# SensorsINI/v2e

Hardware: AMD Instinct MI355X
Metric: Mevents/s (EventEmulator.generate_events, 346x260, 10x slowdown) (higher is better)
Workload: dtype f64

## Files before the change

v2e_amd/csrc/emu.hip:

```cpp
#include "common.h"
#include "../../include/v2e_detmath.h"

#include <cstdarg>
#include <cstdlib>
#include <chrono>
#include <vector>

namespace {

constexpr int BLOCK = 256;
constexpr int WAVE = 64;
constexpr int RING = 64;
constexpr int SCAN_BLOCKS = 64;
constexpr int STAMP_LAUNCHES = 128;

constexpr uint32_t CNT_MASK = 0x00FFFFFFu;
constexpr uint32_t CNT_NEG = 1u << 24;
constexpr uint32_t CNT_SHOT_ON = 1u << 25;
constexpr uint32_t CNT_SHOT_OFF = 1u << 26;

struct FrameCtl {
    double t_prev, t_frame;
    double dt_over_tau;
    double shot_base;
// ... 1801 lines not shown
    const RunScratch &r = h->cur();
    const size_t esz = dtype == V2E_DT_U8 ? 1 : (dtype == V2E_DT_F32 ? 4 : 8);
    const bool has_refr = p->refractory_period_s > 0;
    const int K = h->ch_K, E = h->ch_E, m = E / K, D = h->ch_D, NC = h->n_clips, nD = h->ch_nD;
    const bool fused_rec = h->ch_fused != 0;
    const std::vector<ChainLaunch> plan = chain_plan(n_frames, K, E, nD, has_refr, fused_rec);
    const int nL = (int)plan.size();
    const int nB = (n_frames + K - 1) / K;
    const int nEB = (n_frames + E - 1) / E;
    KArgs a = a_in;
    Sched sc;
    sc.h = h; sc.st[ST_MAIN] = s; sc.st[ST_AHEAD] = h->ahead; sc.st[ST_SIDE] = h->side; sc.st[ST_TAB] = h->tabs; sc.st[ST_SIDE2] = h->side2;
    if (mode == ChainMode::profiled)
        for (int q = 0; q < ST_COUNT; ++q) sc.st[q] = s;
    auto mark = [&](bool rows, hipStream_t stq) -> int {
        if (mode != ChainMode::profiled) return 0;
        hipEvent_t e;
        V2E_HIP(hipEventCreate(&e));
        (rows ? marks->rows : marks->chain).push_back(e);
        V2E_HIP(hipEventRecord(e, stq));
        return 0;
    };
    int gy = NC;
    if (has_refr && K > 1) gy = std::max(1, std::min(NC, h->ch_max_blocks / std::max(h->ngroups, 1)));
    dim3 grid(h->ngroups, gy);
    const int tab_stream = captured || pipelined ? ST_SIDE : ST_TAB;
    constexpr int NSET = 3;
    auto launch_emission = [&](int b, int ef0, int enE) -> int {
        CEmitArgs ea;
        memset(&ea, 0, sizeof(ea));
        ea.ctl = r.run_ctl; ea.recs = recs; ea.fidx_base = r.run_fidx;
        ea.f0 = ef0; ea.nE = enE; ea.D = D; ea.n_clips = NC; ea.slot0 = ef0 % D;
        ea.nwp = h->ch_nwp; ea.nwaves = chain_egroups(h); ea.E = E;
        ea.cnt = r.ch_cnt; ea.tsold = has_refr ? r.ch_tsold : nullptr; ea.ruleM = has_refr ? r.ch_ruleM : nullptr;
        const size_t set = (size_t)(b % NSET) * E * NC;
        ea.wmax = r.ch_wmax + set * h->ch_nwp; ea.wtot = r.ch_wtot + set * h->nkeys_cap * h->ch_nwp;
        ea.cf = r.ch_cf + set; ea.cT = r.ch_cT + set * h->nkeys_cap; ea.ckbase = r.ch_ckbase + set * h->nkeys_cap;
        ea.cperm = r.ch_cperm + set * h->max_iters * 8; ea.cpre = r.ch_cpre + set * h->nkeys_cap * h->ch_nwp;
        ea.cdone = r.ch_cdone + set;
        const bool pull = r.ch_cmask != nullptr;
        ea.cmask = pull ? r.ch_cmask + set * h->ch_nwp * h->nkeys_cap * 2 * GPX : nullptr;
        bool two = h->ch_nwp > 1024;
        if (const char *ev = getenv("V2E_AMD_PULL_TWO_LEVEL")) two = atoi(ev) != 0;
        ea.cpre16 = pull && two ? r.ch_cpre16 + set * h->nkeys_cap * (h->ch_nwp / 16) : nullptr;
        ea.wpf = std::max(4, std::min(two ? 128 : 64, h->npx / (two ? 2048 : V2E_PULL_PX_PER_WG)));
        ea.p2 = two ? 16 : 64;
        while (ea.p2 < (two ? h->ch_nwp / 16 : ea.nwaves)) ea.p2 *= 2;
        ea.events = (float4 *)events; ea.cap = cap;
        ea.off_in = r.run_off + (size_t)b * NC;
        ea.off_out = r.run_off + (size_t)(b + 1) * NC;
        ea.ich = 4;
        ea.capw = GROUP_PX * ea.ich;
        ea.coff_in_cemit = captured || pipelined ? 1 : 0;
        ea.zpw_tot = CTOT_ZF;
        ea.zpw_emit = 1;
        const int REC_LDS = (ea.capw + WAVE) * 4 * (BLOCK / WAVE);
        const int egx = (chain_egroups(h) + BLOCK / WAVE - 1) / (BLOCK / WAVE);
        void *args[] = {(void *)&a, (void *)&ea};
        if (sc.wait(tab_stream, EV_FORK, b)) return V2E_EHIP;
        if (b >= NSET && !captured && sc.wait(tab_stream, EV_JOIN, b - NSET)) return V2E_EHIP;
        if (sc.kernel(tab_stream, (const void *)k_ctot, dim3(egx, NC, (ea.nE + CTOT_ZF - 1) / CTOT_ZF), dim3(BLOCK), 0, args)) return V2E_EHIP;
        if (h->ch_nwp <= 4096) {
            if (sc.kernel(tab_stream, (const void *)k_cframe1, dim3(1, NC, ea.nE), dim3(CFRAME_THREADS), 0, args)) return V2E_EHIP;
        } else if (sc.kernel(tab_stream, (const void *)k_cframe, dim3(std::min(h->nkeys_cap, CFRAME_ROWS), NC, ea.nE), dim3(CFRAME_THREADS), 0, args)) {
            return V2E_EHIP;
        }
        const int row_stream = pipelined ? ST_SIDE2 : captured ? ST_SIDE : ((b & 1) ? ST_SIDE2 : ST_SIDE);
        if (!ea.coff_in_cemit) {
            void *oargs[] = {(void *)&ea};
            if (sc.kernel(tab_stream, (const void *)k_coff, dim3(NC), dim3(WAVE), 0, oargs)) return V2E_EHIP;
        }
        if (sc.record(EV_TAB, b, tab_stream)) return V2E_EHIP;
        if (!captured && sc.wait(row_stream, EV_TAB, b)) return V2E_EHIP;
        if (mark(true, sc.st[row_stream])) return V2E_EHIP;
        if (pull) {
            if (sc.kernel(row_stream, ea.cpre16 ? (const void *)k_cpull<true> : (const void *)k_cpull<false>, dim3(8 * ea.wpf * ((ea.nE + 7) / 8), NC), dim3(BLOCK), (size_t)(2 * ea.p2 * (ea.cpre16 ? 4 : 6)), args)) return V2E_EHIP;
        } else if (sc.kernel(row_stream, (const void *)k_cemit, dim3(egx, NC, ea.nE), dim3(BLOCK), (size_t)REC_LDS, args)) return V2E_EHIP;
        if (mark(true, sc.st[row_stream])) return V2E_EHIP;
        return sc.record(EV_JOIN, b, row_stream);
    };
    const bool split0 = m > 1 && n_frames > K && !pipelined;
    const bool ahead_whole = pipelined && !fused_rec && n_frames <= D;
    auto launch_ahead = [&](int b) -> int {
        if (!ahead_whole && b >= nD && sc.wait(ST_AHEAD, EV_CHAIN, (b - nD + 1) * m)) return V2E_EHIP;
        const int b0 = ahead_whole ? 0 : b * E, b1 = ahead_whole ? n_frames : std::min((b + 1) * E, n_frames);
        const int cut = (b == 0 && split0) ? std::min(K, b1) : b1;
        for (int part = 0; part < 2; ++part) {
            const int f0 = part == 0 ? b0 : cut, f1 = part == 0 ? cut : b1;
            if (f1 <= f0) continue;
            AheadArgs aa;
            memset(&aa, 0, sizeof(aa));
            aa.frames_pp = r.run_frames; aa.frame_stride = (unsigned long long)NC * h->npx * esz;
            aa.ctl = r.run_ctl; aa.fidx_base = r.run_fidx;
            aa.f0 = f0; aa.nf = f1 - f0; aa.D = D; aa.n_clips = NC; aa.slot0 = f0 % D;
            aa.rec = r.ch_rec;
            {
                const int pairs = aa.nf / 2 + 1;
                const long long wg_xy = (long long)h->ngroups * NC;
                int zb = (int)std::min<long long>(pairs, std::max<long long>((4ll * h->n_cu + wg_xy - 1) / wg_xy, (pairs + 15) / 16));
                aa.ppt = (pairs + zb - 1) / zb;
            }
            void *args[] = {(void *)&a, (void *)&aa};
            if (sc.kernel(ST_AHEAD, (const void *)k_ahead<uint8_t>, dim3(h->ngroups, NC, (aa.nf / 2 + 1 + aa.ppt - 1) / aa.ppt), dim3(BLOCK), 0, args)) return V2E_EHIP;
            if (sc.record(EV_AHEAD, part == 0 ? b : nL, ST_AHEAD)) return V2E_EHIP;
        }
        return 0;
    };
    void *xb[2] = {h->base, has_refr ? h->ch_base2 : h->base}, *xl[2] = {h->lp, has_refr ? h->ch_lp2 : h->lp};
    float *xt[2] = {h->ts_mem, has_refr ? h->ch_ts2 : h->ts_mem};
    {
        void *const zp[4] = {recs, r.run_off, has_refr ? (void *)r.ch_gM : nullptr, has_refr ? (void *)r.ch_bar : nullptr};
        const size_t zb[4] = {sizeof(v2e_frame_rec) * (size_t)n_frames * NC, sizeof(unsigned long long) * NC,
                              sizeof(uint32_t) * (size_t)nL * (K + 1) * NC * K, sizeof(unsigned) * (size_t)nL * 2 * K * NC};
        if (sc.zero4(pipelined ? ST_AHEAD : ST_MAIN, zp, zb)) return V2E_EHIP;
    }
    if (!pipelined) {
        if (sc.record(EV_FORK, nL, ST_MAIN)) return V2E_EHIP;
        if (!captured && sc.wait(ST_SIDE, EV_FORK, nL)) return V2E_EHIP;
        if (!fused_rec && sc.wait(ST_AHEAD, EV_FORK, nL)) return V2E_EHIP;
// ... 570 lines not shown
```

v2e_amd/csrc/emu_chain.h:

```cpp
#pragma once
#include <type_traits>
#include "pull_index.h"

#ifndef V2E_CHAIN_LOCKSTEP
#define V2E_CHAIN_LOCKSTEP 0
#endif
#ifndef V2E_CHAIN_STAMPS
#define V2E_CHAIN_STAMPS 0
#endif

constexpr int CHAIN_K_MAX = 64;
constexpr int CFRAME_THREADS = 1024;
constexpr int CHAIN_SUB = 8;
constexpr int CHAIN_MAX_ITERS = 1024;

template <typename R> __device__ __forceinline__ R floor_div_pos(R a, R b)
{
    if (!(b > (R)0) || !(a >= (R)0)) return div_floor<R>(a, b);
    if (a < b) return (R)0;
    R q = floor(a / b);
    R r = fma(-q, b, a);
    if (r < (R)0) q -= (R)1;
    else if (r >= b) q += (R)1;
    return q;
}

__device__ __forceinline__ bool clip_barrier(unsigned *ctr, unsigned target, bool light = false)
{
    __shared__ int s_ok;
    asm volatile("s_waitcnt vmcnt(0)" ::: "memory");
    __syncthreads();
    if (threadIdx.x == 0) {
        if (!light) {
            __builtin_amdgcn_fence(__ATOMIC_RELEASE, "agent");
            asm volatile("s_waitcnt vmcnt(0)" ::: "memory");
        }
        __hip_atomic_fetch_add(ctr, 1u, __ATOMIC_RELAXED, __HIP_MEMORY_SCOPE_AGENT);
        unsigned spins = 0;
        int ok = 1;
        while (__hip_atomic_load(ctr, __ATOMIC_RELAXED, __HIP_MEMORY_SCOPE_AGENT) < target) {
            if (light) __builtin_amdgcn_s_sleep(1); else __builtin_amdgcn_s_sleep(4);
            if (++spins > 2000000u) { ok = 0; break; }
        }
        if (!light) __builtin_amdgcn_fence(__ATOMIC_ACQUIRE, "agent");
        s_ok = ok;
    }
    __syncthreads();
    return s_ok != 0;
}

struct FrameTab {
    float start, step, end;
    uint32_t refr_mask;
    __device__ __forceinline__ FrameTab(const FrameCtl *c, int lane)
        : start(c->ts_start[lane & 31]), step(c->ts_stepf[lane & 31]), end(c->ts_end), refr_mask(c->refr_mask) {}
// ... 616 lines not shown
                if (lane >= c0 && lane < fn) WT_STORE(&ca.ruleM[(size_t)sl * ca.n_clips + clip], rule_v);
            }
            if (own) break;
            if (valid) {
                ((R *)ca.base_fix)[sp] = b;
                if (lp_state) ((R *)ca.lp_fix)[sp] = lp;
                ca.ts_fix[sp] = tsm;
            }
            if (last_exact >= ca.pnf - 1) continue;
            __builtin_amdgcn_s_setprio(0);
            const bool ok = clip_barrier(ca.bar_prev + (size_t)bar_idx * ca.n_clips + clip, (unsigned)ca.ngroups, ca.bar_light != 0);
            ++bar_idx;
            if (ca.prio) __builtin_amdgcn_s_setprio(3);
            if (!ok && tid == 0) atomicOr(&ca.recs[(size_t)ca.pf0 * ca.n_clips + clip].flags, V2E_FLAG_SYNC_TIMEOUT);
        }
        if (valid && (ca.nf > 0 || ca.store_out || redone)) {
            ((R *)ca.base_out)[sp] = b;
            if (ca.nf > 0 || lp_state) ((R *)ca.lp_out)[sp] = lp;
            if (a.has_refr) ca.ts_out[sp] = tsm;
        }
        V2E_STAMP_C(15);
    }
    if (stamp && tid == 0) atomicMax(stamp + 2 * ca.lidx + 1, wall_clock64());
}

struct CFrame {
    int M;
    uint32_t n_events, n_signal, discarded;
};

struct CEmitArgs {
    const FrameCtl *ctl;
    v2e_frame_rec *recs;
    const uint32_t *fidx_base;
    int f0, nE, D, n_clips, nwp, nwaves, E;
    int slot0;
    const uint32_t *cnt;
    const uint32_t *ruleM;
    uint16_t *wmax;
    uint16_t *wtot;
    const float *tsold;
    CFrame *cf;
    uint32_t *cT;
    uint32_t *ckbase;
    uint32_t *cperm;
    uint32_t *cpre;
    float4 *events;
    unsigned long long cap;
    const unsigned long long *off_in;
    unsigned long long *off_out;
    unsigned *cdone;
    int capw, ich;
    int zpw_tot, zpw_emit;
    int coff_in_cemit;
    uint32_t *cmask;
    int wpf, p2;
    uint32_t *cpre16;
};

#ifndef V2E_GPX
#define V2E_GPX 4
#endif
constexpr int GPX = V2E_GPX;
constexpr int GROUP_PX = GPX * WAVE;
constexpr int GROUP_SRC_BITS = GPX <= 4 ? 8 : (GPX <= 8 ? 9 : 10);

constexpr int CTOT_ZF = 2;

__global__ __launch_bounds__(BLOCK) void k_ctot(KArgs a, CEmitArgs ea)
{
    const int tid = threadIdx.x, lane = tid & (WAVE - 1), wave = tid / WAVE;
    const int clip = blockIdx.y;
    const int grp = blockIdx.x * (BLOCK / WAVE) + wave;
    if (grp >= ea.nwaves) return;
    const int p0 = grp * GROUP_PX + lane;
    const int zb = (int)blockIdx.z * CTOT_ZF;
    uint32_t cwq[CTOT_ZF][GPX], rMq[CTOT_ZF];
    int slotq[CTOT_ZF];
    {
        int sl = ea.slot0 + zb;
        if (sl >= ea.D) sl -= ea.D;
#pragma unroll
        for (int q = 0; q < CTOT_ZF; ++q) {
            slotq[q] = sl;
            rMq[q] = 0u;
#pragma unroll
            for (int j = 0; j < GPX; ++j) {
                cwq[q][j] = 0u;
                if (zb + q < ea.nE && p0 + j * WAVE < a.npx) cwq[q][j] = ea.cnt[((size_t)sl * ea.n_clips + clip) * a.npx_pad + p0 + j * WAVE];
            }
            if (zb + q < ea.nE && ea.ruleM) rMq[q] = ea.ruleM[(size_t)sl * ea.n_clips + clip];
            if (++sl == ea.D) sl = 0;
        }
    }
#pragma unroll
    for (int q = 0; q < CTOT_ZF; ++q) {
        const int z = zb + q;
        if (z >= ea.nE) break;
        const size_t zc = (size_t)z * ea.n_clips + clip;
        const uint32_t rM = (uint32_t)__builtin_amdgcn_readfirstlane((int)rMq[q]);
        int magv[GPX];
        bool neg[GPX];
        unsigned long long negb[GPX];
        int mmax = 0;
        uint32_t son = 0, soff = 0;
        unsigned long long sob[GPX], sfb[GPX];
#pragma unroll
        for (int j = 0; j < GPX; ++j) {
            const uint32_t cw = cwq[q][j];
            magv[j] = (int)(cw & CNT_MASK);
            neg[j] = (cw & CNT_NEG) != 0;
            negb[j] = __ballot(neg[j]);
            mmax = max(mmax, magv[j]);
            sob[j] = __ballot((cw & CNT_SHOT_ON) != 0);
            sfb[j] = __ballot((cw & CNT_SHOT_OFF) != 0);
            son += (uint32_t)__popcll(sob[j]);
            soff += (uint32_t)__popcll(sfb[j]);
        }
        const int wm = wave_max_i32(mmax);
        if (lane == 0) ea.wmax[zc * ea.nwp + grp] = (uint16_t)min(wm, 65535);
        uint16_t *trow = ea.wtot + (zc * a.nkeys_cap) * ea.nwp + grp;
        uint32_t *mrow = ea.cmask ? ea.cmask + ((zc * a.nkeys_cap + (lane >= 2 * GPX ? 1 : 0)) * ea.nwp + grp) * (2 * GPX) + (lane & (2 * GPX - 1)) : nullptr;
        auto put_masks = [&](const int key_on, const unsigned long long (&on_m)[GPX], const unsigned long long (&off_m)[GPX]) __attribute__((always_inline)) {
            uint32_t mw = 0u;
#pragma unroll
            for (int j = 0; j < GPX; ++j) {
                asm("v_writelane_b32 %0, %1, %2" : "+v"(mw) : "s"((uint32_t)on_m[j]), "n"(2 * j));
                asm("v_writelane_b32 %0, %1, %2" : "+v"(mw) : "s"((uint32_t)(on_m[j] >> 32)), "n"(2 * j + 1));
                asm("v_writelane_b32 %0, %1, %2" : "+v"(mw) : "s"((uint32_t)off_m[j]), "n"(2 * GPX + 2 * j));
                asm("v_writelane_b32 %0, %1, %2" : "+v"(mw) : "s"((uint32_t)(off_m[j] >> 32)), "n"(2 * GPX + 2 * j + 1));
            }
            if (lane < 4 * GPX) mrow[(size_t)key_on * ea.nwp * (2 * GPX)] = mw;
        };
        static_assert(4 * GPX == 16, "k_ctot: the mask words of an iteration are one 16-lane DPP row");
        uint32_t pmask = 0u;
        if (mrow) {
#pragma unroll
            for (int j = 0; j < GPX; ++j) {
                asm("v_writelane_b32 %0, %1, %2" : "+v"(pmask) : "s"((uint32_t)negb[j]), "n"(2 * j));
                asm("v_writelane_b32 %0, %1, %2" : "+v"(pmask) : "s"((uint32_t)(negb[j] >> 32)), "n"(2 * j + 1));
                asm("v_writelane_b32 %0, %1, %2" : "+v"(pmask) : "s"((uint32_t)negb[j]), "n"(2 * GPX + 2 * j));
                asm("v_writelane_b32 %0, %1, %2" : "+v"(pmask) : "s"((uint32_t)(negb[j] >> 32)), "n"(2 * GPX + 2 * j + 1));
            }
            pmask = lane < 2 * GPX ? ~pmask : (lane < 4 * GPX ? pmask : 0u);
        }
        const int wmc = min(wm, a.max_iters);
        const int nkw = 2 + 2 * wmc;
        bool ruled = false;
        TsGen tg(0.f, 0.f, 0.f, 1);
        float tsm[GPX];
#pragma unroll
        for (int j = 0; j < GPX; ++j) tsm[j] = 0.f;
        if (rM != 0u) {
            const FrameCtl *c = ea.ctl + (size_t)(ea.f0 + z) * ea.n_clips + clip;
            const FrameTab ftb(c, lane);
            tg = frame_tsgen(a, c, ftb, (int)rM, ruled);
            if (ea.tsold) {
#pragma unroll
                for (int j = 0; j < GPX; ++j)
                    if (p0 + j * WAVE < a.npx) tsm[j] = ea.tsold[((size_t)slotq[q] * ea.n_clips + clip) * a.npx_pad + p0 + j * WAVE];
            }
        }
        for (int kb = 0; kb < nkw; kb += WAVE) {
            uint32_t mine = 0;
            const int i_lo = kb == 0 ? 0 : (kb - 2) / 2;
            const int i_hi = min((kb + WAVE - 2) / 2, wmc);
            uint32_t *mrow_i = mrow ? mrow + (size_t)(2 + 2 * i_lo) * ea.nwp * (2 * GPX) : nullptr;
            for (int i = i_lo; i < i_hi; ++i) {
                unsigned long long cb[GPX];
                if (!ruled) {
#pragma unroll
                    for (int j = 0; j < GPX; ++j) cb[j] = __ballot(magv[j] > i);
                } else {
#pragma unroll
                    for (int j = 0; j < GPX; ++j) {
                        bool pass = magv[j] > i;
                        if (pass) {
                            const float t = tg(i);
                            const float pt = 1.0f * t - tsm[j];
                            pass = pt > a.refr_f;
                            if (pass) tsm[j] = t;
                        }
                        cb[j] = __ballot(pass);
                    }
                }
                uint32_t on, off;
                if (mrow) {
                    uint32_t mw = 0u;
#pragma unroll
                    for (int j = 0; j < GPX; ++j) {
                        asm("v_writelane_b32 %0, %1, %2" : "+v"(mw) : "s"((uint32_t)cb[j]), "n"(2 * j));
                        asm("v_writelane_b32 %0, %1, %2" : "+v"(mw) : "s"((uint32_t)(cb[j] >> 32)), "n"(2 * j + 1));
                    }
                    mw = (uint32_t)__builtin_amdgcn_update_dpp((int)mw, (int)mw, 0x118, 0xf, 0xc, false) & pmask;
                    if (lane < 4 * GPX) *mrow_i = mw;
                    mrow_i += (size_t)2 * ea.nwp * (2 * GPX);
                    int c = __popc(mw);
                    c += V2E_DPP(c, 0x111);
                    c += V2E_DPP(c, 0x112);
                    c += V2E_DPP(c, 0x114);
                    on = (uint32_t)__builtin_amdgcn_readlane(c, 2 * GPX - 1);
                    off = (uint32_t)__builtin_amdgcn_readlane(c, 4 * GPX - 1);
                } else {
                    on = 0u;
                    off = 0u;
#pragma unroll
                    for (int j = 0; j < GPX; ++j) {
                        on += (uint32_t)__popcll(cb[j] & ~negb[j]);
                        off += (uint32_t)__popcll(cb[j] & negb[j]);
                    }
                }
                const int kl = 2 + 2 * i - kb;
                if (lane == kl) mine = on;
                if (lane == kl + 1) mine = off;
            }
            if (kb == 0) {
                if (lane == 0) mine = son;
                if (lane == 1) mine = soff;
                if (mrow && (son | soff) != 0u) put_masks(0, sob, sfb);
            }
            if (kb + lane < nkw) trow[(size_t)(kb + lane) * ea.nwp] = (uint16_t)mine;
        }
    }
}

__device__ __forceinline__ void key_row16(const uint16_t *__restrict__ row_at, const uint16_t *__restrict__ wm_at, uint32_t k, uint32_t v[16])
{
    const uint4 t0 = *(const uint4 *)row_at, t1 = *(const uint4 *)(row_at + 8);
    const uint4 m0 = *(const uint4 *)wm_at, m1 = *(const uint4 *)(wm_at + 8);
    const uint32_t tw[8] = {t0.x, t0.y, t0.z, t0.w, t1.x, t1.y, t1.z, t1.w};
    const uint32_t mw[8] = {m0.x, m0.y, m0.z, m0.w, m1.x, m1.y, m1.z, m1.w};
#pragma unroll
    for (int j = 0; j < 16; ++j) {
        const uint32_t wmj = (mw[j >> 1] >> (16 * (j & 1))) & 0xFFFFu;
        v[j] = k < 2u + 2u * wmj ? ((tw[j >> 1] >> (16 * (j & 1))) & 0xFFFFu) : 0u;
    }
}

__global__ __launch_bounds__(CFRAME_THREADS) void k_cframe1(KArgs a, CEmitArgs ea)
{
    __shared__ int s_red[CFRAME_THREADS / WAVE];
    __shared__ uint32_t s_T[2 * CHAIN_MAX_ITERS + 2];
    constexpr int NW = CFRAME_THREADS / WAVE;
    const int tid = threadIdx.x, lane = tid & (WAVE - 1), wave = tid / WAVE;
    const int clip = blockIdx.y, z = blockIdx.z, fe = ea.f0 + z;
    const uint16_t *wm = ea.wmax + ((size_t)z * ea.n_clips + clip) * ea.nwp;
    int m = 0;
    for (int k = tid; k < ea.nwaves; k += CFRAME_THREADS) m = max(m, (int)wm[k]);
    m = wave_max_i32(m);
    if (lane == 0) s_red[wave] = m;
    __syncthreads();
    int M = 0;
#pragma unroll
    for (int q = 0; q < NW; ++q) M = max(M, s_red[q]);
    M = __builtin_amdgcn_readfirstlane(M);
    CFrame *cf = ea.cf + (size_t)z * ea.n_clips + clip;
    v2e_frame_rec *rec = ea.recs + (size_t)fe * ea.n_clips + clip;
    if (M > a.max_iters) {
        if (tid == 0) {
            cf->M = M; cf->n_events = 0u; cf->n_signal = 0u; cf->discarded = 1u;
            rec->max_events = M;
            atomicOr(&rec->flags, V2E_FLAG_ITERS_CLAMPED);
        }
        return;
    }
    const int nk = 2 + 2 * M;
    const uint16_t *tot = ea.wtot + ((size_t)z * ea.n_clips + clip) * a.nkeys_cap * ea.nwp;
    uint32_t *pre = ea.cpre + ((size_t)z * ea.n_clips + clip) * a.nkeys_cap * ea.nwp;
    for (int k = wave; k < nk; k += NW) {
        uint32_t carry = 0;
        for (int w0 = 0; w0 < ea.nwp; w0 += 16 * WAVE) {
            const int wi = w0 + lane * 16;
            uint32_t v[16];
#pragma unroll
            for (int j = 0; j < 16; ++j) v[j] = 0u;
            if (wi < ea.nwp) {
                key_row16(tot + (size_t)k * ea.nwp + wi, wm + wi, (uint32_t)k, v);
            }
            uint32_t lane_tot = 0;
#pragma unroll
            for (int j = 0; j < 16; ++j) lane_tot += v[j];
            uint32_t run = carry + wave_excl_scan_u32(lane_tot, lane);
            carry += wave_sum_u32(lane_tot);
            if (wi < ea.nwp) {
                uint32_t o[16];
#pragma unroll
                for (int j = 0; j < 16; ++j) { o[j] = run; run += v[j]; }
                uint4 *dst = (uint4 *)(pre + (size_t)k * ea.nwp + wi);
                if (ea.cpre16) ea.cpre16[(((size_t)z * ea.n_clips + clip) * a.nkeys_cap + k) * (ea.nwp / 16) + wi / 16] = o[0];
                dst[0] = make_uint4(o[0], o[1], o[2], o[3]);
                dst[1] = make_uint4(o[4], o[5], o[6], o[7]);
                dst[2] = make_uint4(o[8], o[9], o[10], o[11]);
                dst[3] = make_uint4(o[12], o[13], o[14], o[15]);
            }
        }
        if (lane == 0) s_T[k] = carry;
    }
    __syncthreads();
    if (wave != 0) return;
    uint32_t *cT = ea.cT + ((size_t)z * ea.n_clips + clip) * a.nkeys_cap;
    uint32_t *ckb = ea.ckbase + ((size_t)z * ea.n_clips + clip) * a.nkeys_cap;
    uint32_t carry = 0, sum_on = 0, sum_off = 0;
    for (int kb = 0; kb < nk; kb += WAVE) {
        const int key = kb + lane;
        const uint32_t T_k = key < nk ? s_T[key] : 0u;
        const uint32_t sig = key >= 2 ? T_k : 0u;
        const uint32_t kbase = carry + wave_excl_scan_u32(sig, lane);
        if (key < a.nkeys_cap) { cT[key] = T_k; ckb[key] = kbase; }
        sum_on += wave_sum_u32((lane & 1) ? 0u : sig);
        sum_off += wave_sum_u32((lane & 1) ? sig : 0u);
        carry += wave_sum_u32(sig);
    }
    const uint32_t n_signal = carry;
    uint32_t *perm = ea.cperm + ((size_t)z * ea.n_clips + clip) * a.max_iters * 8;
    if (a.shuffle && a.rng_mode == V2E_RNG_PHILOX) {
        const uint32_t fbase = ea.fidx_base ? *ea.fidx_base : 0u;
        for (int i = lane; i < M; i += WAVE) {
            uint32_t pk[4], sh, aa, amask;
            const uint32_t n_i = s_T[2 + 2 * i] + s_T[3 + 2 * i];
            v2e_perm_shape(n_i, &sh, &aa, &amask);
            v2e_perm_keys(a.seed, (uint32_t)clip, fbase + (uint32_t)fe, (uint32_t)i, pk);
            uint4 *pp = (uint4 *)(perm + (size_t)i * 8);
            pp[0] = make_uint4(pk[0], pk[1], pk[2], pk[3]);
            pp[1] = make_uint4(sh, aa, amask, n_i);
        }
    }
    if (lane == 0) {
        const uint32_t son = a.do_shot ? s_T[0] : 0u, soff = a.do_shot ? s_T[1] : 0u;
        cf->M = M; cf->n_signal = n_signal; cf->n_events = n_signal + son + soff; cf->discarded = 0u;
        rec->max_events = M;
        rec->n_signal = n_signal;
        rec->n_events = n_signal + son + soff;
        rec->n_on = sum_on + son;
        rec->n_off = sum_off + soff;
    }
}

constexpr int CFRAME_ROWS = 24;

__global__ __launch_bounds__(CFRAME_THREADS) void k_cframe(KArgs a, CEmitArgs ea)
{
    constexpr int NW = CFRAME_THREADS / WAVE;
    __shared__ int s_red[NW];
    __shared__ uint32_t s_seg[NW];
    __shared__ uint32_t s_T[2 * CHAIN_MAX_ITERS + 2];
    __shared__ int s_last;
    const int tid = threadIdx.x, lane = tid & (WAVE - 1), wave = tid / WAVE;
    const int r0 = blockIdx.x, clip = blockIdx.y, z = blockIdx.z, fe = ea.f0 + z;
    const size_t zc = (size_t)z * ea.n_clips + clip;
    const uint16_t *wm = ea.wmax + ((size_t)z * ea.n_clips + clip) * ea.nwp;
    int m = 0;
    for (int k = tid; k < ea.nwaves; k += CFRAME_THREADS) m = max(m, (int)wm[k]);
    m = wave_max_i32(m);
    if (lane == 0) s_red[wave] = m;
    __syncthreads();
    int M = 0;
#pragma unroll
    for (int q = 0; q < NW; ++q) M = max(M, s_red[q]);
    M = __builtin_amdgcn_readfirstlane(M);
    CFrame *cf = ea.cf + zc;
    v2e_frame_rec *rec = ea.recs + (size_t)fe * ea.n_clips + clip;
    const bool discard = M > a.max_iters;
    const int nk = discard ? 0 : 2 + 2 * M;
    const uint16_t *tot = ea.wtot + ((size_t)z * ea.n_clips + clip) * a.nkeys_cap * ea.nwp;
    uint32_t *pre = ea.cpre + zc * a.nkeys_cap * ea.nwp;
    uint32_t *cT = ea.cT + zc * a.nkeys_cap;
    const int seg = ((ea.nwp + NW - 1) / NW + 15) / 16 * 16;
    for (int k = r0; k < nk; k += (r0 == (int)gridDim.x - 1 ? 1 : nk)) {
        const int lo = wave * seg, hi = min(lo + seg, ea.nwp);
        uint32_t wsum = 0;
        for (int w0 = lo; w0 < hi; w0 += 16 * WAVE) {
            const int wi = w0 + lane * 16;
            uint32_t lane_tot = 0;
            if (wi < hi) {
                uint32_t v[16];
                key_row16(tot + (size_t)k * ea.nwp + wi, wm + wi, (uint32_t)k, v);
#pragma unroll
                for (int j = 0; j < 16; ++j) lane_tot += v[j];
            }
            wsum += wave_sum_u32(lane_tot);
        }
        __syncthreads();
        if (lane == 0) s_seg[wave] = wsum;
        __syncthreads();
        uint32_t carry = 0, total = 0;
#pragma unroll
        for (int q = 0; q < NW; ++q) {
// ... 475 lines not shown
```

Baseline: 20120.

## Fuse per-frame table build into k_ctot via last-arrival counter and adaptive z-chunking

```diff
diff --git a/v2e_amd/csrc/ctot_walk.h b/v2e_amd/csrc/ctot_walk.h
--- /dev/null
+++ b/v2e_amd/csrc/ctot_walk.h
@@ -0,0 +1,23 @@
+#pragma once
+
+#if defined(__HIPCC__)
+#define V2E_CW_HD __host__ __device__ __forceinline__
+#else
+#define V2E_CW_HD static inline
+#endif
+
+#define CTOT_WG_GROUPS 4
+
+V2E_CW_HD int ctot_arrivals(int nwaves) { return (nwaves + CTOT_WG_GROUPS - 1) / CTOT_WG_GROUPS; }
+V2E_CW_HD int ctot_chunks(int nE, int zf) { return (nE + zf - 1) / zf; }
+V2E_CW_HD int ctot_chunk_frames(int nE, int zf, int c) { return nE - c * zf < zf ? nE - c * zf : zf; }
+V2E_CW_HD int ctot_slot(int slot0, int z, int D) { return slot0 + z >= D ? slot0 + z - D : slot0 + z; }
+V2E_CW_HD int ctot_next_slot(int sl, int D) { return sl + 1 == D ? 0 : sl + 1; }
+
+#define CTOT_ZF_MAX 16
+V2E_CW_HD int ctot_plan_zf(long long wgs_xy, int nE, int n_cu)
+{
+    int zf = CTOT_ZF_MAX;
+    while (zf > 1 && wgs_xy * ctot_chunks(nE, zf) < (long long)n_cu) zf /= 2;
+    return zf;
+}
diff --git a/v2e_amd/csrc/emu.hip b/v2e_amd/csrc/emu.hip
--- a/v2e_amd/csrc/emu.hip
+++ b/v2e_amd/csrc/emu.hip
@@ -1877,19 +1877,17 @@
         ea.ich = 4;
         ea.capw = GROUP_PX * ea.ich;
         ea.coff_in_cemit = captured || pipelined ? 1 : 0;
-        ea.zpw_tot = CTOT_ZF;
+        const int egx = ctot_arrivals(chain_egroups(h));
+        ea.zpw_tot = ctot_plan_zf((long long)egx * NC, ea.nE, h->n_cu);
+        if (const char *ev = getenv("V2E_AMD_CTOT_ZF")) { const int v = atoi(ev); if (v >= 1 && v <= 64) ea.zpw_tot = v; }
+        ea.fuse_frame = h->ch_nwp <= 4096 ? 1 : 0;
         ea.zpw_emit = 1;
         const int REC_LDS = (ea.capw + WAVE) * 4 * (BLOCK / WAVE);
-        const int egx = (chain_egroups(h) + BLOCK / WAVE - 1) / (BLOCK / WAVE);
         void *args[] = {(void *)&a, (void *)&ea};
         if (sc.wait(tab_stream, EV_FORK, b)) return V2E_EHIP;
         if (b >= NSET && !captured && sc.wait(tab_stream, EV_JOIN, b - NSET)) return V2E_EHIP;
-        if (sc.kernel(tab_stream, (const void *)k_ctot, dim3(egx, NC, (ea.nE + CTOT_ZF - 1) / CTOT_ZF), dim3(BLOCK), 0, args)) return V2E_EHIP;
-        if (h->ch_nwp <= 4096) {
-            if (sc.kernel(tab_stream, (const void *)k_cframe1, dim3(1, NC, ea.nE), dim3(CFRAME_THREADS), 0, args)) return V2E_EHIP;
-        } else if (sc.kernel(tab_stream, (const void *)k_cframe, dim3(std::min(h->nkeys_cap, CFRAME_ROWS), NC, ea.nE), dim3(CFRAME_THREADS), 0, args)) {
-            return V2E_EHIP;
-        }
+        if (sc.kernel(tab_stream, (const void *)k_ctot, dim3(egx, NC, ctot_chunks(ea.nE, ea.zpw_tot)), dim3(BLOCK), 0, args)) return V2E_EHIP;
+        if (!ea.fuse_frame && sc.kernel(tab_stream, (const void *)k_cframe, dim3(std::min(h->nkeys_cap, CFRAME_ROWS), NC, ea.nE), dim3(CFRAME_THREADS), 0, args)) return V2E_EHIP;
         const int row_stream = pipelined ? ST_SIDE2 : captured ? ST_SIDE : ((b & 1) ? ST_SIDE2 : ST_SIDE);
         if (!ea.coff_in_cemit) {
             void *oargs[] = {(void *)&ea};
diff --git a/v2e_amd/csrc/emu_chain.h b/v2e_amd/csrc/emu_chain.h
--- a/v2e_amd/csrc/emu_chain.h
+++ b/v2e_amd/csrc/emu_chain.h
@@ -1,6 +1,7 @@
 #pragma once
 #include <type_traits>
 #include "pull_index.h"
+#include "ctot_walk.h"
 
 #ifndef V2E_CHAIN_LOCKSTEP
 #define V2E_CHAIN_LOCKSTEP 0
@@ -723,6 +724,7 @@
     unsigned *cdone;
     int capw, ich;
     int zpw_tot, zpw_emit;
+    int fuse_frame;
     int coff_in_cemit;
     uint32_t *cmask;
     int wpf, p2;
@@ -736,165 +738,6 @@
 constexpr int GROUP_PX = GPX * WAVE;
 constexpr int GROUP_SRC_BITS = GPX <= 4 ? 8 : (GPX <= 8 ? 9 : 10);
 
-constexpr int CTOT_ZF = 2;
-
-__global__ __launch_bounds__(BLOCK) void k_ctot(KArgs a, CEmitArgs ea)
-{
-    const int tid = threadIdx.x, lane = tid & (WAVE - 1), wave = tid / WAVE;
-    const int clip = blockIdx.y;
-    const int grp = blockIdx.x * (BLOCK / WAVE) + wave;
-    if (grp >= ea.nwaves) return;
-    const int p0 = grp * GROUP_PX + lane;
-    const int zb = (int)blockIdx.z * CTOT_ZF;
-    uint32_t cwq[CTOT_ZF][GPX], rMq[CTOT_ZF];
-    int slotq[CTOT_ZF];
-    {
-        int sl = ea.slot0 + zb;
-        if (sl >= ea.D) sl -= ea.D;
-#pragma unroll
-        for (int q = 0; q < CTOT_ZF; ++q) {
-            slotq[q] = sl;
-            rMq[q] = 0u;
-#pragma unroll
-            for (int j = 0; j < GPX; ++j) {
-                cwq[q][j] = 0u;
-                if (zb + q < ea.nE && p0 + j * WAVE < a.npx) cwq[q][j] = ea.cnt[((size_t)sl * ea.n_clips + clip) * a.npx_pad + p0 + j * WAVE];
-            }
-            if (zb + q < ea.nE && ea.ruleM) rMq[q] = ea.ruleM[(size_t)sl * ea.n_clips + clip];
-            if (++sl == ea.D) sl = 0;
-        }
-    }
-#pragma unroll
-    for (int q = 0; q < CTOT_ZF; ++q) {
-        const int z = zb + q;
-        if (z >= ea.nE) break;
-        const size_t zc = (size_t)z * ea.n_clips + clip;
-        const uint32_t rM = (uint32_t)__builtin_amdgcn_readfirstlane((int)rMq[q]);
-        int magv[GPX];
-        bool neg[GPX];
-        unsigned long long negb[GPX];
-        int mmax = 0;
-        uint32_t son = 0, soff = 0;
-        unsigned long long sob[GPX], sfb[GPX];
-#pragma unroll
-        for (int j = 0; j < GPX; ++j) {
-            const uint32_t cw = cwq[q][j];
-            magv[j] = (int)(cw & CNT_MASK);
-            neg[j] = (cw & CNT_NEG) != 0;
-            negb[j] = __ballot(neg[j]);
-            mmax = max(mmax, magv[j]);
-            sob[j] = __ballot((cw & CNT_SHOT_ON) != 0);
-            sfb[j] = __ballot((cw & CNT_SHOT_OFF) != 0);
-            son += (uint32_t)__popcll(sob[j]);
-            soff += (uint32_t)__popcll(sfb[j]);
-        }
-        const int wm = wave_max_i32(mmax);
-        if (lane == 0) ea.wmax[zc * ea.nwp + grp] = (uint16_t)min(wm, 65535);
-        uint16_t *trow = ea.wtot + (zc * a.nkeys_cap) * ea.nwp + grp;
-        uint32_t *mrow = ea.cmask ? ea.cmask + ((zc * a.nkeys_cap + (lane >= 2 * GPX ? 1 : 0)) * ea.nwp + grp) * (2 * GPX) + (lane & (2 * GPX - 1)) : nullptr;
-        auto put_masks = [&](const int key_on, const unsigned long long (&on_m)[GPX], const unsigned long long (&off_m)[GPX]) __attribute__((always_inline)) {
-            uint32_t mw = 0u;
-#pragma unroll
-            for (int j = 0; j < GPX; ++j) {
-                asm("v_writelane_b32 %0, %1, %2" : "+v"(mw) : "s"((uint32_t)on_m[j]), "n"(2 * j));
-                asm("v_writelane_b32 %0, %1, %2" : "+v"(mw) : "s"((uint32_t)(on_m[j] >> 32)), "n"(2 * j + 1));
-                asm("v_writelane_b32 %0, %1, %2" : "+v"(mw) : "s"((uint32_t)off_m[j]), "n"(2 * GPX + 2 * j));
-                asm("v_writelane_b32 %0, %1, %2" : "+v"(mw) : "s"((uint32_t)(off_m[j] >> 32)), "n"(2 * GPX + 2 * j + 1));
-            }
-            if (lane < 4 * GPX) mrow[(size_t)key_on * ea.nwp * (2 * GPX)] = mw;
-        };
-        static_assert(4 * GPX == 16, "k_ctot: the mask words of an iteration are one 16-lane DPP row");
-        uint32_t pmask = 0u;
-        if (mrow) {
-#pragma unroll
-            for (int j = 0; j < GPX; ++j) {
-                asm("v_writelane_b32 %0, %1, %2" : "+v"(pmask) : "s"((uint32_t)negb[j]), "n"(2 * j));
-                asm("v_writelane_b32 %0, %1, %2" : "+v"(pmask) : "s"((uint32_t)(negb[j] >> 32)), "n"(2 * j + 1));
-                asm("v_writelane_b32 %0, %1, %2" : "+v"(pmask) : "s"((uint32_t)negb[j]), "n"(2 * GPX + 2 * j));
-                asm("v_writelane_b32 %0, %1, %2" : "+v"(pmask) : "s"((uint32_t)(negb[j] >> 32)), "n"(2 * GPX + 2 * j + 1));
-            }
-            pmask = lane < 2 * GPX ? ~pmask : (lane < 4 * GPX ? pmask : 0u);
-        }
-        const int wmc = min(wm, a.max_iters);
-        const int nkw = 2 + 2 * wmc;
-        bool ruled = false;
-        TsGen tg(0.f, 0.f, 0.f, 1);
-        float tsm[GPX];
-#pragma unroll
-        for (int j = 0; j < GPX; ++j) tsm[j] = 0.f;
-        if (rM != 0u) {
-            const FrameCtl *c = ea.ctl + (size_t)(ea.f0 + z) * ea.n_clips + clip;
-            const FrameTab ftb(c, lane);
-            tg = frame_tsgen(a, c, ftb, (int)rM, ruled);
-            if (ea.tsold) {
-#pragma unroll
-                for (int j = 0; j < GPX; ++j)
-                    if (p0 + j * WAVE < a.npx) tsm[j] = ea.tsold[((size_t)slotq[q] * ea.n_clips + clip) * a.npx_pad + p0 + j * WAVE];
-            }
-        }
-        for (int kb = 0; kb < nkw; kb += WAVE) {
-            uint32_t mine = 0;
-            const int i_lo = kb == 0 ? 0 : (kb - 2) / 2;
-            const int i_hi = min((kb + WAVE - 2) / 2, wmc);
-            uint32_t *mrow_i = mrow ? mrow + (size_t)(2 + 2 * i_lo) * ea.nwp * (2 * GPX) : nullptr;
-            for (int i = i_lo; i < i_hi; ++i) {
-                unsigned long long cb[GPX];
-                if (!ruled) {
-#pragma unroll
-                    for (int j = 0; j < GPX; ++j) cb[j] = __ballot(magv[j] > i);
-                } else {
-#pragma unroll
-                    for (int j = 0; j < GPX; ++j) {
-                        bool pass = magv[j] > i;
-                        if (pass) {
-                            const float t = tg(i);
-                            const float pt = 1.0f * t - tsm[j];
-                            pass = pt > a.refr_f;
-                            if (pass) tsm[j] = t;
-                        }
-                        cb[j] = __ballot(pass);
-                    }
-                }
-                uint32_t on, off;
-                if (mrow) {
-                    uint32_t mw = 0u;
-#pragma unroll
-                    for (int j = 0; j < GPX; ++j) {
-                        asm("v_writelane_b32 %0, %1, %2" : "+v"(mw) : "s"((uint32_t)cb[j]), "n"(2 * j));
-                        asm("v_writelane_b32 %0, %1, %2" : "+v"(mw) : "s"((uint32_t)(cb[j] >> 32)), "n"(2 * j + 1));
-                    }
-                    mw = (uint32_t)__builtin_amdgcn_update_dpp((int)mw, (int)mw, 0x118, 0xf, 0xc, false) & pmask;
-                    if (lane < 4 * GPX) *mrow_i = mw;
-                    mrow_i += (size_t)2 * ea.nwp * (2 * GPX);
-                    int c = __popc(mw);
-                    c += V2E_DPP(c, 0x111);
-                    c += V2E_DPP(c, 0x112);
-                    c += V2E_DPP(c, 0x114);
-                    on = (uint32_t)__builtin_amdgcn_readlane(c, 2 * GPX - 1);
-                    off = (uint32_t)__builtin_amdgcn_readlane(c, 4 * GPX - 1);
-                } else {
-                    on = 0u;
-                    off = 0u;
-#pragma unroll
-                    for (int j = 0; j < GPX; ++j) {
-                        on += (uint32_t)__popcll(cb[j] & ~negb[j]);
-                        off += (uint32_t)__popcll(cb[j] & negb[j]);
-                    }
-                }
-                const int kl = 2 + 2 * i - kb;
-                if (lane == kl) mine = on;
-                if (lane == kl + 1) mine = off;
-            }
-            if (kb == 0) {
-                if (lane == 0) mine = son;
-                if (lane == 1) mine = soff;
-                if (mrow && (son | soff) != 0u) put_masks(0, sob, sfb);
-            }
-            if (kb + lane < nkw) trow[(size_t)(kb + lane) * ea.nwp] = (uint16_t)mine;
-        }
-    }
-}
-
 __device__ __forceinline__ void key_row16(const uint16_t *__restrict__ row_at, const uint16_t *__restrict__ wm_at, uint32_t k, uint32_t v[16])
 {
     const uint4 t0 = *(const uint4 *)row_at, t1 = *(const uint4 *)(row_at + 8);
@@ -908,16 +751,15 @@
     }
 }
 
-__global__ __launch_bounds__(CFRAME_THREADS) void k_cframe1(KArgs a, CEmitArgs ea)
-{
-    __shared__ int s_red[CFRAME_THREADS / WAVE];
-    __shared__ uint32_t s_T[2 * CHAIN_MAX_ITERS + 2];
-    constexpr int NW = CFRAME_THREADS / WAVE;
+__device__ __forceinline__ void ctot_frame_tables(const KArgs &a, const CEmitArgs &ea, const int z, const int clip, int *s_red)
+{
+    constexpr int NW = BLOCK / WAVE;
     const int tid = threadIdx.x, lane = tid & (WAVE - 1), wave = tid / WAVE;
-    const int clip = blockIdx.y, z = blockIdx.z, fe = ea.f0 + z;
-    const uint16_t *wm = ea.wmax + ((size_t)z * ea.n_clips + clip) * ea.nwp;
+    const int fe = ea.f0 + z;
+    const size_t zc = (size_t)z * ea.n_clips + clip;
+    const uint16_t *wm = ea.wmax + zc * ea.nwp;
     int m = 0;
-    for (int k = tid; k < ea.nwaves; k += CFRAME_THREADS) m = max(m, (int)wm[k]);
+    for (int k = tid; k < ea.nwaves; k += BLOCK) m = max(m, (int)wm[k]);
     m = wave_max_i32(m);
     if (lane == 0) s_red[wave] = m;
     __syncthreads();
@@ -925,7 +767,7 @@
 #pragma unroll
     for (int q = 0; q < NW; ++q) M = max(M, s_red[q]);
     M = __builtin_amdgcn_readfirstlane(M);
-    CFrame *cf = ea.cf + (size_t)z * ea.n_clips + clip;
+    CFrame *cf = ea.cf + zc;
     v2e_frame_rec *rec = ea.recs + (size_t)fe * ea.n_clips + clip;
     if (M > a.max_iters) {
         if (tid == 0) {
@@ -933,11 +775,13 @@
             rec->max_events = M;
             atomicOr(&rec->flags, V2E_FLAG_ITERS_CLAMPED);
         }
+        __syncthreads();
         return;
     }
     const int nk = 2 + 2 * M;
-    const uint16_t *tot = ea.wtot + ((size_t)z * ea.n_clips + clip) * a.nkeys_cap * ea.nwp;
-    uint32_t *pre = ea.cpre + ((size_t)z * ea.n_clips + clip) * a.nkeys_cap * ea.nwp;
+    const uint16_t *tot = ea.wtot + zc * a.nkeys_cap * ea.nwp;
+    uint32_t *pre = ea.cpre + zc * a.nkeys_cap * ea.nwp;
+    uint32_t *cT = ea.cT + zc * a.nkeys_cap;
     for (int k = wave; k < nk; k += NW) {
         uint32_t carry = 0;
         for (int w0 = 0; w0 < ea.nwp; w0 += 16 * WAVE) {
@@ -945,9 +789,7 @@
             uint32_t v[16];
 #pragma unroll
             for (int j = 0; j < 16; ++j) v[j] = 0u;
-            if (wi < ea.nwp) {
-                key_row16(tot + (size_t)k * ea.nwp + wi, wm + wi, (uint32_t)k, v);
-            }
+            if (wi < ea.nwp) key_row16(tot + (size_t)k * ea.nwp + wi, wm + wi, (uint32_t)k, v);
             uint32_t lane_tot = 0;
 #pragma unroll
             for (int j = 0; j < 16; ++j) lane_tot += v[j];
@@ -958,52 +800,251 @@
 #pragma unroll
                 for (int j = 0; j < 16; ++j) { o[j] = run; run += v[j]; }
                 uint4 *dst = (uint4 *)(pre + (size_t)k * ea.nwp + wi);
-                if (ea.cpre16) ea.cpre16[(((size_t)z * ea.n_clips + clip) * a.nkeys_cap + k) * (ea.nwp / 16) + wi / 16] = o[0];
+                if (ea.cpre16) ea.cpre16[(zc * a.nkeys_cap + k) * (ea.nwp / 16) + wi / 16] = o[0];
                 dst[0] = make_uint4(o[0], o[1], o[2], o[3]);
                 dst[1] = make_uint4(o[4], o[5], o[6], o[7]);
                 dst[2] = make_uint4(o[8], o[9], o[10], o[11]);
                 dst[3] = make_uint4(o[12], o[13], o[14], o[15]);
             }
         }
-        if (lane == 0) s_T[k] = carry;
+        if (lane == 0) cT[k] = carry;
     }
     __syncthreads();
-    if (wave != 0) return;
-    uint32_t *cT = ea.cT + ((size_t)z * ea.n_clips + clip) * a.nkeys_cap;
-    uint32_t *ckb = ea.ckbase + ((size_t)z * ea.n_clips + clip) * a.nkeys_cap;
-    uint32_t carry = 0, sum_on = 0, sum_off = 0;
-    for (int kb = 0; kb < nk; kb += WAVE) {
-        const int key = kb + lane;
-        const uint32_t T_k = key < nk ? s_T[key] : 0u;
-        const uint32_t sig = key >= 2 ? T_k : 0u;
-        const uint32_t kbase = carry + wave_excl_scan_u32(sig, lane);
-        if (key < a.nkeys_cap) { cT[key] = T_k; ckb[key] = kbase; }
-        sum_on += wave_sum_u32((lane & 1) ? 0u : sig);
-        sum_off += wave_sum_u32((lane & 1) ? sig : 0u);
-        carry += wave_sum_u32(sig);
-    }
-    const uint32_t n_signal = carry;
-    uint32_t *perm = ea.cperm + ((size_t)z * ea.n_clips + clip) * a.max_iters * 8;
-    if (a.shuffle && a.rng_mode == V2E_RNG_PHILOX) {
-        const uint32_t fbase = ea.fidx_base ? *ea.fidx_base : 0u;
-        for (int i = lane; i < M; i += WAVE) {
-            uint32_t pk[4], sh, aa, amask;
-            const uint32_t n_i = s_T[2 + 2 * i] + s_T[3 + 2 * i];
-            v2e_perm_shape(n_i, &sh, &aa, &amask);
-            v2e_perm_keys(a.seed, (uint32_t)clip, fbase + (uint32_t)fe, (uint32_t)i, pk);
-            uint4 *pp = (uint4 *)(perm + (size_t)i * 8);
-            pp[0] = make_uint4(pk[0], pk[1], pk[2], pk[3]);
-            pp[1] = make_uint4(sh, aa, amask, n_i);
-        }
-    }
-    if (lane == 0) {
-        const uint32_t son = a.do_shot ? s_T[0] : 0u, soff = a.do_shot ? s_T[1] : 0u;
-        cf->M = M; cf->n_signal = n_signal; cf->n_events = n_signal + son + soff; cf->discarded = 0u;
-        rec->max_events = M;
-        rec->n_signal = n_signal;
-        rec->n_events = n_signal + son + soff;
-        rec->n_on = sum_on + son;
-        rec->n_off = sum_off + soff;
+    if (wave == 0) {
+        uint32_t *ckb = ea.ckbase + zc * a.nkeys_cap;
+        uint32_t carry = 0, sum_on = 0, sum_off = 0;
+        uint32_t shot_on = 0, shot_off = 0;
+        for (int kb = 0; kb < nk; kb += WAVE) {
+            const int key = kb + lane;
+            const uint32_t T_k = key < nk ? cT[key] : 0u;
+            const uint32_t sig = key >= 2 ? T_k : 0u;
+            const uint32_t kbase = carry + wave_excl_scan_u32(sig, lane);
+            if (key >= nk && key < a.nkeys_cap) cT[key] = 0u;
+            if (key < a.nkeys_cap) ckb[key] = kbase;
+            if (kb == 0) {
+                shot_on = (uint32_t)__builtin_amdgcn_readlane((int)T_k, 0);
+                shot_off = (uint32_t)__builtin_amdgcn_readlane((int)T_k, 1);
+            }
+            sum_on += wave_sum_u32((lane & 1) ? 0u : sig);
+            sum_off += wave_sum_u32((lane & 1) ? sig : 0u);
+            carry += wave_sum_u32(sig);
+        }
+        const uint32_t n_signal = carry;
+        uint32_t *perm = ea.cperm + zc * a.max_iters * 8;
+        if (a.shuffle && a.rng_mode == V2E_RNG_PHILOX) {
+            const uint32_t fbase = ea.fidx_base ? *ea.fidx_base : 0u;
+            for (int i = lane; i < M; i += WAVE) {
+                uint32_t pk[4], sh, aa, amask;
+                const uint32_t n_i = cT[2 + 2 * i] + cT[3 + 2 * i];
+                v2e_perm_shape(n_i, &sh, &aa, &amask);
+                v2e_perm_keys(a.seed, (uint32_t)clip, fbase + (uint32_t)fe, (uint32_t)i, pk);
+                uint4 *pp = (uint4 *)(perm + (size_t)i * 8);
+                pp[0] = make_uint4(pk[0], pk[1], pk[2], pk[3]);
+                pp[1] = make_uint4(sh, aa, amask, n_i);
+            }
+        }
+        if (lane == 0) {
+            const uint32_t son = a.do_shot ? shot_on : 0u, soff = a.do_shot ? shot_off : 0u;
+            cf->M = M; cf->n_signal = n_signal; cf->n_events = n_signal + son + soff; cf->discarded = 0u;
+            rec->max_events = M;
+            rec->n_signal = n_signal;
+            rec->n_events = n_signal + son + soff;
+            rec->n_on = sum_on + son;
+            rec->n_off = sum_off + soff;
+        }
+    }
+    __syncthreads();
+}
+
+__global__ __launch_bounds__(BLOCK) void k_ctot(KArgs a, CEmitArgs ea)
+{
+    __shared__ int s_red[BLOCK / WAVE];
+    __shared__ int s_last[2];
+    const int tid = threadIdx.x, lane = tid & (WAVE - 1), wave = tid / WAVE;
+    const int clip = blockIdx.y;
+    static_assert(CTOT_WG_GROUPS == BLOCK / WAVE, "ctot_walk.h: a k_ctot workgroup's groups are its waves");
+    const int grp = blockIdx.x * CTOT_WG_GROUPS + wave;
+    const bool live = grp < ea.nwaves;
+    const bool fuse = ea.fuse_frame != 0;
+    if (!live && !fuse) return;
+    const int zb = (int)blockIdx.z * ea.zpw_tot;
+    const int nz = ctot_chunk_frames(ea.nE, ea.zpw_tot, (int)blockIdx.z);
+    const int p0 = grp * GROUP_PX + lane;
+    bool inb[GPX];
+#pragma unroll
+    for (int j = 0; j < GPX; ++j) inb[j] = live && p0 + j * WAVE < a.npx;
+    int sl = ctot_slot(ea.slot0, zb, ea.D);
+    const size_t fstride = (size_t)ea.n_clips * a.npx_pad;
+    const size_t sp0 = ((size_t)sl * ea.n_clips + clip) * a.npx_pad + p0;
+    const uint32_t *cp = ea.cnt + sp0;
+    const float *tp = ea.tsold ? ea.tsold + sp0 : nullptr;
+    const uint32_t *rp = ea.ruleM ? ea.ruleM + (size_t)sl * ea.n_clips + clip : nullptr;
+    const size_t zc0 = (size_t)zb * ea.n_clips + clip;
+    const size_t tstride = (size_t)ea.n_clips * a.nkeys_cap * ea.nwp;
+    uint16_t *wmp = ea.wmax + zc0 * ea.nwp + grp;
+    uint16_t *trow = ea.wtot + zc0 * a.nkeys_cap * ea.nwp + grp;
+    uint32_t *mrow = ea.cmask ? ea.cmask + ((zc0 * a.nkeys_cap + (lane >= 2 * GPX ? 1 : 0)) * ea.nwp + grp) * (2 * GPX) + (lane & (2 * GPX - 1)) : nullptr;
+    const FrameCtl *ctl = ea.ctl + (size_t)(ea.f0 + zb) * ea.n_clips + clip;
+    unsigned *done = ea.cdone + zc0;
+    const unsigned last_old = (unsigned)ctot_arrivals(ea.nwaves) - 1u;
+    uint32_t cw[GPX], rM = 0u;
+#pragma unroll
+    for (int j = 0; j < GPX; ++j) cw[j] = inb[j] ? cp[j * WAVE] : 0u;
+    if (rp) rM = *rp;
+    unsigned old_prev = 0u;
+    for (int q = 0; q < nz + (fuse ? 1 : 0); ++q) {
+        uint32_t cwn[GPX], rMn = 0u;
+        const int sln = ctot_next_slot(sl, ea.D);
+        const bool wrap = sln != sl + 1;
+        const uint32_t *cpn = wrap ? cp - (size_t)(ea.D - 1) * fstride : cp + fstride;
+        const uint32_t *rpn = rp ? (wrap ? rp - (size_t)(ea.D - 1) * ea.n_clips : rp + ea.n_clips) : nullptr;
+        const float *tpn = tp ? (wrap ? tp - (size_t)(ea.D - 1) * fstride : tp + fstride) : nullptr;
+#pragma unroll
+        for (int j = 0; j < GPX; ++j) cwn[j] = (q + 1 < nz && inb[j]) ? cpn[j * WAVE] : 0u;
+        if (q + 1 < nz && rpn) rMn = *rpn;
+        if (live && q < nz) {
+            rM = (uint32_t)__builtin_amdgcn_readfirstlane((int)rM);
+            int magv[GPX];
+            unsigned long long negb[GPX];
+            int mmax = 0;
+            uint32_t son = 0, soff = 0;
+            unsigned long long sob[GPX], sfb[GPX];
+#pragma unroll
+            for (int j = 0; j < GPX; ++j) {
+                magv[j] = (int)(cw[j] & CNT_MASK);
+                negb[j] = __ballot((cw[j] & CNT_NEG) != 0);
+                mmax = max(mmax, magv[j]);
+                sob[j] = __ballot((cw[j] & CNT_SHOT_ON) != 0);
+                sfb[j] = __ballot((cw[j] & CNT_SHOT_OFF) != 0);
+                son += (uint32_t)__popcll(sob[j]);
+                soff += (uint32_t)__popcll(sfb[j]);
+            }
+            const int wm = wave_max_i32(mmax);
+            if (lane == 0) *wmp = (uint16_t)min(wm, 65535);
+            auto put_masks = [&](const int key_on, const unsigned long long (&on_m)[GPX], const unsigned long long (&off_m)[GPX]) __attribute__((always_inline)) {
+                uint32_t mw = 0u;
+#pragma unroll
+                for (int j = 0; j < GPX; ++j) {
+                    asm("v_writelane_b32 %0, %1, %2" : "+v"(mw) : "s"((uint32_t)on_m[j]), "n"(2 * j));
+                    asm("v_writelane_b32 %0, %1, %2" : "+v"(mw) : "s"((uint32_t)(on_m[j] >> 32)), "n"(2 * j + 1));
+                    asm("v_writelane_b32 %0, %1, %2" : "+v"(mw) : "s"((uint32_t)off_m[j]), "n"(2 * GPX + 2 * j));
+                    asm("v_writelane_b32 %0, %1, %2" : "+v"(mw) : "s"((uint32_t)(off_m[j] >> 32)), "n"(2 * GPX + 2 * j + 1));
+                }
+                if (lane < 4 * GPX) mrow[(size_t)key_on * ea.nwp * (2 * GPX)] = mw;
+            };
+            static_assert(4 * GPX == 16, "k_ctot: the mask words of an iteration are one 16-lane DPP row");
+            uint32_t pmask = 0u;
+            if (mrow) {
+#pragma unroll
+                for (int j = 0; j < GPX; ++j) {
+                    asm("v_writelane_b32 %0, %1, %2" : "+v"(pmask) : "s"((uint32_t)negb[j]), "n"(2 * j));
+                    asm("v_writelane_b32 %0, %1, %2" : "+v"(pmask) : "s"((uint32_t)(negb[j] >> 32)), "n"(2 * j + 1));
+                    asm("v_writelane_b32 %0, %1, %2" : "+v"(pmask) : "s"((uint32_t)negb[j]), "n"(2 * GPX + 2 * j));
+                    asm("v_writelane_b32 %0, %1, %2" : "+v"(pmask) : "s"((uint32_t)(negb[j] >> 32)), "n"(2 * GPX + 2 * j + 1));
+                }
+                pmask = lane < 2 * GPX ? ~pmask : (lane < 4 * GPX ? pmask : 0u);
+            }
+            const int wmc = min(wm, a.max_iters);
+            const int nkw = 2 + 2 * wmc;
+            bool ruled = false;
+            TsGen tg(0.f, 0.f, 0.f, 1);
+            float tsm[GPX];
+#pragma unroll
+            for (int j = 0; j < GPX; ++j) tsm[j] = 0.f;
+            if (rM != 0u) {
+                const FrameTab ftb(ctl, lane);
+                tg = frame_tsgen(a, ctl, ftb, (int)rM, ruled);
+                if (tp) {
+#pragma unroll
+                    for (int j = 0; j < GPX; ++j)
+                        if (inb[j]) tsm[j] = tp[j * WAVE];
+                }
+            }
+            for (int kb = 0; kb < nkw; kb += WAVE) {
+                uint32_t mine = 0;
+                const int i_lo = kb == 0 ? 0 : (kb - 2) / 2;
+                const int i_hi = min((kb + WAVE - 2) / 2, wmc);
+                uint32_t *mrow_i = mrow ? mrow + (size_t)(2 + 2 * i_lo) * ea.nwp * (2 * GPX) : nullptr;
+                for (int i = i_lo; i < i_hi; ++i) {
+                    unsigned long long cb[GPX];
+                    if (!ruled) {
+#pragma unroll
+                        for (int j = 0; j < GPX; ++j) cb[j] = __ballot(magv[j] > i);
+                    } else {
+#pragma unroll
+                        for (int j = 0; j < GPX; ++j) {
+                            bool pass = magv[j] > i;
+                            if (pass) {
+                                const float t = tg(i);
+                                const float pt = 1.0f * t - tsm[j];
+                                pass = pt > a.refr_f;
+                                if (pass) tsm[j] = t;
+                            }
+                            cb[j] = __ballot(pass);
+                        }
+                    }
+                    uint32_t on, off;
+                    if (mrow) {
+                        uint32_t mw = 0u;
+#pragma unroll
+                        for (int j = 0; j < GPX; ++j) {
+                            asm("v_writelane_b32 %0, %1, %2" : "+v"(mw) : "s"((uint32_t)cb[j]), "n"(2 * j));
+                            asm("v_writelane_b32 %0, %1, %2" : "+v"(mw) : "s"((uint32_t)(cb[j] >> 32)), "n"(2 * j + 1));
+                        }
+                        mw = (uint32_t)__builtin_amdgcn_update_dpp((int)mw, (int)mw, 0x118, 0xf, 0xc, false) & pmask;
+                        if (lane < 4 * GPX) *mrow_i = mw;
+                        mrow_i += (size_t)2 * ea.nwp * (2 * GPX);
+                        int c = __popc(mw);
+                        c += V2E_DPP(c, 0x111);
+                        c += V2E_DPP(c, 0x112);
+                        c += V2E_DPP(c, 0x114);
+                        on = (uint32_t)__builtin_amdgcn_readlane(c, 2 * GPX - 1);
+                        off = (uint32_t)__builtin_amdgcn_readlane(c, 4 * GPX - 1);
+                    } else {
+                        on = 0u;
+                        off = 0u;
+#pragma unroll
+                        for (int j = 0; j < GPX; ++j) {
+                            on += (uint32_t)__popcll(cb[j] & ~negb[j]);
+                            off += (uint32_t)__popcll(cb[j] & negb[j]);
+                        }
+                    }
+                    const int kl = 2 + 2 * i - kb;
+                    if (lane == kl) mine = on;
+                    if (lane == kl + 1) mine = off;
+                }
+                if (kb == 0) {
+                    if (lane == 0) mine = son;
+                    if (lane == 1) mine = soff;
+                    if (mrow && (son | soff) != 0u) put_masks(0, sob, sfb);
+                }
+                if (kb + lane < nkw) trow[(size_t)(kb + lane) * ea.nwp] = (uint16_t)mine;
+            }
+        }
+        if (fuse) {
+            if (tid == 0) s_last[q & 1] = q > 0 && old_prev == last_old;
+            __syncthreads();
+            if (tid == 0 && q < nz) {
+                __builtin_amdgcn_fence(__ATOMIC_RELEASE, "agent");
+                unsigned lane_off = 0u;
+                asm volatile("" : "+v"(lane_off));
+                old_prev = __hip_atomic_fetch_add(done + (size_t)q * ea.n_clips + lane_off, 1u, __ATOMIC_RELAXED, __HIP_MEMORY_SCOPE_AGENT);
+            }
+            if (s_last[q & 1]) {
+                __builtin_amdgcn_fence(__ATOMIC_ACQUIRE, "agent");
+                if (tid == 0) __hip_atomic_store(done + (size_t)(q - 1) * ea.n_clips, 0u, __ATOMIC_RELAXED, __HIP_MEMORY_SCOPE_AGENT);
+                ctot_frame_tables(a, ea, zb + q - 1, clip, s_red);
+            }
+        }
+#pragma unroll
+        for (int j = 0; j < GPX; ++j) cw[j] = cwn[j];
+        rM = rMn;
+        cp = cpn; rp = rpn; tp = tpn;
+        sl = sln;
+        wmp += (size_t)ea.n_clips * ea.nwp;
+        trow += tstride;
+        if (mrow) mrow += tstride * (2 * GPX);
+        ctl += ea.n_clips;
     }
 }
 
```

Measured after the change: 5989. 0.298x the previous value.
